# ArchDD/CPP-Raytracer-Rasterizer

Measured on AMD Instinct MI355X. Metric: Mrays/s (primary+shadow), higher is better.
Workload: dtype f32

## Files before the change

cpp-raytracer-rasterizer_amd/capi/binned.cpp:

```cpp
#include "capi.hpp"

namespace mirt {


int PairList::ensure(size_t cap)
{
    int r;
    if ((r = dev_realloc(&d_entries, cap)) || (r = dev_realloc(&d_pair_keys, cap)) || (r = dev_realloc(&d_pair_vals, cap)) ||
        (r = dev_realloc(&d_sorted_keys, cap)) || (r = dev_realloc(&d_tmp_vals, cap))) { cap_entries = 0; return r; }
    cap_entries = (uint32_t)cap;
    return MIRT_OK;
}


void PairList::poll()
{
    if (count_pending && hipEventQuery(ev_count) == hipSuccess) {
        known_pairs = *h_count; have_known = true; count_pending = false;
    }
    (void)hipGetLastError();
}

int PairList::record_count()
{
    if (!count_event_due) return MIRT_OK;
    count_event_due = false;
    HIP_TRY(hipEventRecord(ev_count, g.stream));
    count_pending = true;
    return MIRT_OK;
}

PassPlan KeptPass::plan_for(uint64_t key, int mode, PairList &P) const
{
    static const bool reuse_off = env_int("MIRT_BIN_REUSE", 1) == 0;
    P.poll();
    return kept_pass_plan(bin_key_valid, bin_key == key, P.have_known, P.known_pairs > P.cap_used, last_bin_mode == mode, reuse_off);
}

int bin_pass(PairList &S, BinSet bs, const OriginRow *cam_tab, const OriginRow *light_tab, uint32_t *counter, uint32_t *bin_off,
             uint32_t *npairs, bool may_guess = false)
{
    int rc;
    S.count_event_due = false;
    S.poll();
    const bool guess = may_guess && S.have_known;
    if (!S.d_entries || !S.cap_entries) {
        static const size_t initial = [] { const long v = env_int("MIRT_BIN_INITIAL_PAIRS", 0); return v > 0 ? (size_t)v : (size_t)1 << 20; }();
        if ((rc = S.ensure(initial))) return rc;
    }
    if (bs.nbins > BIN_MAX_KEYS) return fail(MIRT_ERR_INVALID_ARGUMENT, "binning: %u sort keys exceed the %u the bucket sort holds", bs.nbins, BIN_MAX_KEYS);
    bs.chunk_tris = 256;
    const dim3 bin_grid((unsigned)std::min<long long>((long long)((g.n + bs.chunk_tris - 1) / bs.chunk_tris) * bs.nframes, (long long)g.cu_count * 8));
    bs.counters = counter;
    const uint32_t nbuckets = bucket_sort_buckets(bs.nbins);
    if (nbuckets + 1 > S.cap_buckets) {
        if ((rc = dev_grow(&S.d_bucket, &S.cap_buckets, nbuckets + 1, (size_t)3 * (nbuckets + 1), false))) return rc;
        HIP_TRY(hipMemsetAsync(S.d_bucket, 0, sizeof(uint32_t) * 3 * (nbuckets + 1), g.stream));
        S.bucket_dirty = false;
    }
    uint32_t *bcnt = S.d_bucket, *bbase = S.d_bucket + S.cap_buckets, *bcur = S.d_bucket + 2 * (size_t)S.cap_buckets;
    bs.bucket_cnt = bcnt; bs.nbuckets = nbuckets; bs.bucket_shift = bucket_sort_shift(bs.nbins);
    const size_t bin_lds = (size_t)nbuckets * sizeof(uint32_t);
    {
        static const bool once = [] {
            (void)hipFuncSetAttribute(reinterpret_cast<const void *>(&k_bin_pairs<512>), hipFuncAttributeMaxDynamicSharedMemorySize, 48 * 1024);
            (void)hipFuncSetAttribute(reinterpret_cast<const void *>(&k_bin_pairs<256>), hipFuncAttributeMaxDynamicSharedMemorySize, 48 * 1024);
            return true; }();
        (void)once;
    }
    static const int bin_wg_env = (int)env_int("MIRT_BIN_WG", 0);
    const int bin_wg = (bin_wg_env == 256 || bin_wg_env == 512) ? bin_wg_env : ((g.n < 400000 && g.in_flight >= 3) ? 256 : 512);
    if (guess && pairs_wanted(S.known_pairs) > S.cap_entries) {
        HIP_TRY(hipStreamSynchronize(g.stream));
        if ((rc = S.ensure(pairs_grown(pairs_wanted(S.known_pairs))))) return rc;
    }
    bool publish_count = false;
    for (int attempt = 0; attempt < 2; attempt++) {
        static const uint32_t test_cap = [] { const long v = env_int("MIRT_TEST_PAIR_CAP", 0); return v > 0 ? (uint32_t)v : 0u; }();
        S.cap_used = (guess && test_cap && test_cap < S.cap_entries) ? test_cap : S.cap_entries;
        BinPairs pairs = { S.d_pair_keys, S.d_pair_vals, S.cap_used };
        bs.entries = S.d_entries; bs.cap_entries = S.cap_used;
        if (attempt) HIP_TRY(hipMemsetAsync(counter, 0, 4, g.stream));
        if (attempt || S.bucket_dirty) HIP_TRY(hipMemsetAsync(S.d_bucket, 0, sizeof(uint32_t) * 3 * (size_t)S.cap_buckets, g.stream));
        S.bucket_dirty = true;
        if (bin_wg == 256) hipLaunchKernelGGL(k_bin_pairs<256>, bin_grid, dim3(256), bin_lds, g.stream, g.d_tris, cam_tab, light_tab, g.n, bs, pairs);
        else hipLaunchKernelGGL(k_bin_pairs<512>, bin_grid, dim3(512), bin_lds, g.stream, g.d_tris, cam_tab, light_tab, g.n, bs, pairs);
        if (guess) {
            if (!S.h_count) {
                HIP_TRY(hipHostMalloc(reinterpret_cast<void **>(&S.h_count), 64, hipHostMallocDefault));
                HIP_TRY(hipEventCreateWithFlags(&S.ev_count, hipEventDisableTiming));
            }
            if (!S.count_pending) publish_count = true;
            *npairs = S.known_pairs;
            break;
        }
        uint32_t total = 0;
        HIP_TRY(hipStreamSynchronize(g.stream));
        HIP_TRY(hipMemcpy(&total, counter, 4, hipMemcpyDeviceToHost));
        *npairs = total;
        S.known_pairs = total; S.have_known = true;
        S.count_pending = false;
        if (total <= S.cap_entries) break;
        if (attempt == 1) return fail(MIRT_ERR_HIP, "binning produced %u pairs twice with room for %u", total, S.cap_entries);
        if ((rc = S.ensure(pairs_after_readback(total)))) return rc;
    }
#ifdef MIRT_BIN_STATS
    {
        uint32_t c[16];
        (void)hipMemcpy(c, counter, 64, hipMemcpyDeviceToHost);
        fprintf(stderr, "[mirt bin stats] flattened units=%u max per work item=%u direct items=%u | huge: box valid=%u no box=%u (camera frame %u) waves in the joint test=%u\n", c[8], c[9], c[10], c[11], c[12], c[14], c[15]);
        fprintf(stderr, "[mirt bin stats] tris=%d frames=%d  pairs=%u  bins=%u | large items walked=%u level-1 rounds=%u level-2 steps=%u pairs=%u max steps/item=%u items>100 steps=%u\n",
                g.n, bs.nframes, *npairs, bs.nbins, c[2], c[3], c[4], c[5], c[6], c[7]);
        (void)hipMemset(counter + 2, 0, 56);
    }
#endif
    uint32_t *count_out = nullptr;
    if (publish_count) HIP_TRY(hipHostGetDevicePointer(reinterpret_cast<void **>(&count_out), S.h_count, 0));
    HIP_TRY(bucket_sort_pairs(S.d_pair_keys, S.d_pair_vals, counter, S.cap_used, *npairs, bs.nbins, S.d_sorted_keys, S.d_tmp_vals,
                              bcnt, bbase, bcur, bin_off, S.d_entries, g.cu_count, g.stream, count_out));
    S.bucket_dirty = false;
    S.count_event_due = publish_count;
    return MIRT_OK;
}

uint64_t light_key_of(const float *origins, int nlights)
{
    return Fnv(g.scene_version).mix(origins + 3, sizeof(float) * 3 * nlights).mix(&nlights, 4).mix(&g.n, 4).h;
}

int light_shells_for(int nlights, int cube_bins, uint32_t keys_in_front)
{
    static const int env = (int)env_int("MIRT_LIGHT_SHELLS", 0);
    return light_shells_rule(nlights, cube_bins, keys_in_front, env);
}

int ensure_face_lists(LightPass &S, int nlights)
{
    int rc;
    if ((rc = S.ensure_counters(LIGHT_COUNTER_BYTES))) return rc;
    S.d_face_counts = S.d_bin_counters + 128;
    const size_t want = (size_t)6 * (size_t)nlights * (size_t)g.n;
    if (want > S.cap_face_sel && (rc = dev_grow(&S.d_face_sel, &S.cap_face_sel, want, want, true))) return rc;
    return MIRT_OK;
}

static int cube_bin_chain(LightPass &S, const BinFrameDesc *d_frames, const float *d_origins, int nlights, uint32_t nkeys, OriginRow *light_tab,
                          uint32_t *bin_off, uint32_t *counter, uint32_t *npairs, bool may_guess)
{
    hipLaunchKernelGGL(k_select_faces, dim3((unsigned)std::min<long long>(((long long)g.n + 1023) / 1024, (long long)g.cu_count), nlights), dim3(1024), 0, g.stream,
                       g.d_tris, g.n, d_origins, d_frames, light_tab, S.d_face_sel, (uint32_t)g.n, S.d_face_counts);
    BinSet bs;
    memset(&bs, 0, sizeof bs);
    bs.frames = d_frames; bs.nframes = 6 * nlights; bs.nbins = nkeys; bs.bin_off = bin_off;
    bs.face_lists = S.d_face_sel; bs.face_counts = S.d_face_counts; bs.face_stride = (uint32_t)g.n;
    return bin_pass(S.pairs, bs, nullptr, light_tab, counter, bin_off, npairs, may_guess);
}

int light_cache_ensure(LightCache &C, LightPass &S, const float *origins, int nlights, int cube_bins, bool *built)
{
    int rc;
    const uint64_t key = light_key_of(origins, nlights);
    if (built) *built = false;
    if (C.holds(key, cube_bins)) return MIRT_OK;
    if (built) *built = true;
// ... 115 lines not shown
    kept.forget();
    return dev_grow(&d_sel, &sel_n, g.n, (size_t)g.n, true);
}

SelectOut CameraPass::select_out(const OriginTables &T, int count_word) const
{
    SelectOut so;
    memset(&so, 0, sizeof so);
    so.cam_tab = T.d_cam_tab; so.sel = d_sel;
    so.sel_count = d_bin_counters + count_word; so.sel_count_next = d_bin_counters + (count_word ^ 1);
    return so;
}

static void launch_prep_select(const BinFrameDesc &frame, const SelectOut &so)
{
    const unsigned sel_grid = (unsigned)std::min<long long>(((long long)g.n + 1023) / 1024, (long long)g.cu_count);
    if (sel_grid) hipLaunchKernelGGL(k_prep_select, dim3(sel_grid), dim3(1024), 0, g.stream, g.d_tris, g.n, frame, so);
}

int binned_pass(const mirt_view *view, StreamState &ss, const float *origins, int nlights, int y0, int y1, BinnedPass *bp)
{
    int rc;
    CameraPass &S = ss.cam;
    LightPass &L = ss.lt;
    g.stats.mode_used = MIRT_RT_BINNED;
    g.stats_sel_count = nullptr;
    bool fixed_grid = false;
    const int fine_bins = light_cube_bins_for(nlights, &fixed_grid);

    const uint64_t lkey = light_key_of(origins, nlights);
    if (g.lc.track_key == lkey) g.lc.stable++;
    else { g.lc.track_key = lkey; g.lc.stable = 0; }
// ... 97 lines not shown
    CameraPass &S = ss.cam;
    if ((rc = ss.tabs.ensure_cam_rows()) || (rc = S.ensure_sel()) || (rc = S.ensure_counters(512))) return rc;
    S.kept.forget();
    const BinFrameDesc fr = make_camera_frame(view, 0, 0, g.aa);
    SelectOut so = S.select_out(ss.tabs, HIST_SEL_COUNT);
    if ((rc = hist_prepare(ss.hist, fr, &so))) return rc;
    if (!g.hist_armed) return MIRT_OK;
    HIP_TRY(hipMemsetAsync(so.sel_count, 0, 4, g.stream));
    launch_prep_select(fr, so);
    HIP_TRY(hipGetLastError());
    return hist_publish(ss.hist);
}

int binned_trace(const RtFrame &f, StreamState &ss, const BinnedPass &bp)
{
    int rc;
    CameraPass &S = ss.cam;
    RtTraceFrame tf;
    memset(&tf, 0, sizeof tf);
    tf.f = f;
    tf.f.cam_tab = ss.tabs.d_cam_tab;
    tf.f.light_tab = bp.light_tab;
    tf.f.unsafe = nullptr;
    tf.cam_off = bp.cam_off;
    tf.cam_entries = S.pairs.d_entries;
    tf.sel = S.d_sel; tf.sel_count = S.d_bin_counters + SEL_COUNT0 + S.sel_parity;
    static const int lazy_env = (int)env_int("MIRT_LAZY_GEO", -1);
    const bool lazy_geo = lazy_env >= 0 ? (lazy_env != 0) : (g.n >= 400000);
    tf.geo = g.d_geo;
    tf.shade = g.d_shade;
    tf.light_off = bp.cube.light_off;
// ... 17 lines not shown
    const size_t lds = rt_trace_lds_bytes(1);
    k_begin(MIRT_K_TRACE);
    g.pending_counted = g.profiling;
    if (f.aa > 1) {
        if (g.profiling) hipLaunchKernelGGL((k_rt_trace2<true, true>), tgrid, dim3(64), lds, g.stream, tf);
        else hipLaunchKernelGGL((k_rt_trace2<true, false>), tgrid, dim3(64), lds, g.stream, tf);
    } else {
        static const int waves5_env = (int)env_int("MIRT_TR_WAVES5", -1);
        const bool waves5 = waves5_env >= 0 ? (waves5_env != 0) : (g.n >= 400000 || g.in_flight <= 2);
        if (g.profiling) hipLaunchKernelGGL((k_rt_trace2<false, true>), tgrid, dim3(64), lds, g.stream, tf);
        else if (waves5) hipLaunchKernelGGL((k_rt_trace2<false, false, 5>), tgrid, dim3(64), lds, g.stream, tf);
        else hipLaunchKernelGGL((k_rt_trace2<false, false>), tgrid, dim3(64), lds, g.stream, tf);
    }
    k_end(MIRT_K_TRACE);
    HIP_TRY(hipGetLastError());
    return (rc = S.pairs.record_count()) ? rc : ss.lt.pairs.record_count();
}

}
```

cpp-raytracer-rasterizer_amd/capi/capi.hpp:

```cpp
#pragma once

#include "../csrc/bin_sort.hpp"
#include "../csrc/comm.hpp"
#include "../csrc/cull.hpp"
#include "../csrc/dof.hpp"
#include "../csrc/rt_common.hpp"
#include "../csrc/raster_common.hpp"
#include "../csrc/rt_binned.hpp"
#include "../csrc/rt_trace_frame.hpp"
#include "../csrc/scan.hpp"
#include "../query/rt_query.hpp"
#include "../lights/many_lights.hpp"
#include "cube_plan.hpp"
#include "pass_plan.hpp"
#include "object_plan.hpp"
#include "dof_plan.hpp"
#include "env.hpp"

#include <cstdarg>
#include <cstdio>
#include <cstdlib>
#include <cstring>
#include <algorithm>
#include <cmath>
// ... 53 lines not shown
    uint32_t *d_flags = nullptr;

    int ensure_cam_rows();
    void release();
};

struct PairList {
    uint32_t *d_entries = nullptr;
    uint32_t *d_pair_keys = nullptr, *d_pair_vals = nullptr, *d_sorted_keys = nullptr;
    uint32_t *d_tmp_vals = nullptr;
    uint32_t *d_bucket = nullptr;
    uint32_t cap_buckets = 0;
    bool bucket_dirty = false;
    uint32_t cap_entries = 0;
    uint32_t cap_used = 0;
    uint32_t *h_count = nullptr;
    hipEvent_t ev_count = nullptr;
    bool count_pending = false;
    bool count_event_due = false;
    bool have_known = false;
    uint32_t known_pairs = 0;

    int ensure(size_t cap);
    void poll();
    int record_count();
    void forget_scene() { have_known = false; count_pending = false; }
    void release();
};

struct KeptPass {
    uint64_t bin_key = 0;
    bool bin_key_valid = false;
    int last_bin_mode = -1;
    uint32_t bin_entries = 0;

    PassPlan plan_for(uint64_t key, int mode, PairList &P) const;
    void keep(uint64_t key, int mode) { bin_key = key; last_bin_mode = mode; bin_key_valid = true; }
    void forget() { bin_key_valid = false; }
};

// ... 424 lines not shown
```

cpp-raytracer-rasterizer_amd/capi/pass_plan.hpp:

```cpp
#pragma once

#include "../query/rt_query.hpp"
#include "cube_plan.hpp"

#include <cmath>
#include <cstring>

namespace mirt {

struct Fnv {
    uint64_t h;
    explicit Fnv(uint64_t seed) : h(0xcbf29ce484222325ull ^ seed) {}
    Fnv &mix(const void *p, size_t nb) { for (size_t i = 0; i < nb; i++) { h ^= ((const unsigned char *)p)[i]; h *= 0x100000001b3ull; } return *this; }
};

struct PassPlan { bool fresh, may_guess, reuse; };
inline PassPlan kept_pass_plan(bool valid, bool key_equal, bool count_known, bool count_above_cap, bool same_kind, bool reuse_off)
{
    const bool fresh = !valid || !key_equal || (count_known && count_above_cap);
    return PassPlan{ fresh, same_kind, !fresh && !reuse_off };
}

inline size_t pairs_wanted(uint32_t known) { return (size_t)known + known / 2 + 4096; }
inline size_t pairs_grown(size_t want) { return want + want / 4; }
inline size_t pairs_after_readback(uint32_t total) { return (size_t)total + total / 8 + 4096; }

inline int light_shells_rule(int nlights, int cube_bins, uint32_t keys_in_front, int env)
{
    const long long bins = 6ll * cube_bins * cube_bins * std::max(nlights, 1);
    int ns = (env >= 1 && env <= 64) ? env : 16;
    while (ns > 1 && bins * ns + keys_in_front + 64 > (long long)BIN_MAX_KEYS) ns >>= 1;
    return ns;
}
inline int camera_shells_rule(long long tiles, int env)
{
    int ns = (int)std::min<long long>(8, std::max<long long>(1, (4ll << 20) / std::max<long long>(tiles, 1)));
    if (env >= 1 && env <= 64) ns = env;
    while (ns > 1 && tiles * ns + 64 > (long long)BIN_MAX_KEYS) ns >>= 1;
    return ns;
}
// ... 60 lines not shown
```

cpp-raytracer-rasterizer_amd/capi/state.cpp:

```cpp
#include "capi.hpp"

namespace mirt {

int dev_realloc_bytes(void **p, size_t bytes)
{
    if (*p) { (void)hipFree(*p); *p = nullptr; }
    if (bytes == 0) return MIRT_OK;
    hipError_t e = hipMalloc(p, bytes);
    if (e != hipSuccess) { *p = nullptr; return fail(MIRT_ERR_OUT_OF_MEMORY, "hipMalloc(%zu bytes): %s", bytes, hipGetErrorString(e)); }
    return MIRT_OK;
}

int check_frame_args(const mirt_view *view, const mirt_light *lights, int nlights, const float *indirect, const void *xrgb, int pitch_bytes,
                     bool need_scene, int y0, int y1)
{
    int rc;
    if ((rc = need_init())) return rc;
    if (!view || !indirect) return fail(MIRT_ERR_INVALID_ARGUMENT, "view / indirect must not be NULL");
    if (view->width < 1 || view->height < 1 || view->width > 32768 || view->height > 32768)
        return fail(MIRT_ERR_INVALID_ARGUMENT, "frame size %dx%d out of range [1,32768]", view->width, view->height);
    if (nlights < 0 || nlights > MIRT_MAX_LIGHTS) return fail(MIRT_ERR_INVALID_ARGUMENT, "nlights %d out of range [0,%d]", nlights, MIRT_MAX_LIGHTS);
    if (nlights > 0 && !lights) return fail(MIRT_ERR_INVALID_ARGUMENT, "lights must not be NULL when nlights > 0");
    if (need_scene && g.n <= 0) return fail(MIRT_ERR_NO_SCENE, "no scene uploaded (mirt_scene_upload)");
    if (!xrgb) return fail(MIRT_ERR_INVALID_ARGUMENT, "xrgb output must not be NULL");
// ... 32 lines not shown
    memset(ss.ev_used, 0, sizeof ss.ev_used);
    ss.call_timed = g.profiling;
    if (ss.call_timed) (void)hipEventRecord(ss.ev[EV_CALL0], g.stream);
}
void call_end() { if (g.cur().call_timed) (void)hipEventRecord(g.cur().ev[EV_CALL1], g.stream); g.stats_stream = g.stream; g.stats_pending = true; }


static void dev_free(std::initializer_list<void *> ptrs) { for (void *p : ptrs) if (p) (void)hipFree(p); }

void OriginTables::release() { dev_free({ d_cam_tab, d_light_tab, d_origins, d_flags }); *this = OriginTables(); }

void PairList::release()
{
    dev_free({ d_entries, d_pair_keys, d_pair_vals, d_sorted_keys, d_tmp_vals, d_bucket });
    if (h_count) (void)hipHostFree(h_count);
    if (ev_count) (void)hipEventDestroy(ev_count);
    *this = PairList();
}

void CameraPass::release() { pairs.release(); dev_free({ d_bin_off, d_bin_counters, d_frames, d_sel, d_order }); *this = CameraPass(); }

void LightPass::release() { pairs.release(); dev_free({ d_bin_off, d_bin_counters, d_frames, d_face_sel, d_light_tab, d_light_rows }); *this = LightPass(); }

void CostHist::release()
{
    dev_free({ d_hist });
    if (h_hist) (void)hipHostFree(h_hist);
    for (hipEvent_t e : ev_hist) if (e) (void)hipEventDestroy(e);
    *this = CostHist();
}

// ... 67 lines not shown
```

cpp-raytracer-rasterizer_amd/csrc/bin_bucket_sort.hip:

```cpp
#include "bin_sort.hpp"

#include <algorithm>
#include <cstdlib>
#include <type_traits>

namespace mirt {

constexpr int BS_PER_THREAD = 16;
constexpr int BS_CHUNK = 256 * BS_PER_THREAD;
constexpr int BS_LOCAL_PER_THREAD = 16;
constexpr int BS_MAX_SHIFT = 12;
constexpr int BS_MAX_BUCKET_KEYS = 1 << BS_MAX_SHIFT;

__device__ __forceinline__ uint32_t bs_block_scan(uint32_t v, uint32_t *s_wave , uint32_t *total)
{
    const int lane = threadIdx.x & 63, wave = threadIdx.x >> 6;
    uint32_t incl = v;
#pragma unroll
    for (int d = 1; d < 64; d <<= 1) {
        const uint32_t o = __shfl_up(incl, d);
        if (lane >= d) incl += o;
    }
    __syncthreads();
    if (lane == 63) s_wave[wave] = incl;
    __syncthreads();
    uint32_t off = 0, all = 0;
#pragma unroll
    for (int w = 0; w < 4; w++) { if (w < wave) off += s_wave[w]; all += s_wave[w]; }
    *total = all;
    return off + incl - v;
}

__global__ __launch_bounds__(256) void k_bs_scatter(const uint32_t *__restrict__ keys, const uint32_t *__restrict__ vals,
                                                    const uint32_t *__restrict__ total_ptr, uint32_t cap, uint32_t nbuckets, int shift,
                                                    const uint32_t *__restrict__ bucket_cnt, uint32_t *__restrict__ bucket_base,
                                                    uint32_t *__restrict__ cursor, uint32_t *__restrict__ out_keys, uint32_t *__restrict__ out_vals,
                                                    uint32_t *__restrict__ count_out)
{
    extern __shared__ uint32_t s_dyn[];
    __shared__ uint32_t s_wave[4];
    if (count_out && blockIdx.x == 0 && threadIdx.x == 0) *count_out = *total_ptr;
    if (*total_ptr > cap) return;
    uint32_t *s_base = s_dyn, *s_cnt = s_dyn + nbuckets;
    uint32_t carry = 0;
    for (uint32_t b0 = 0; b0 < nbuckets; b0 += 256) {
        const uint32_t b = b0 + threadIdx.x;
        const uint32_t c = b < nbuckets ? bucket_cnt[b] : 0u;
        uint32_t all;
        const uint32_t excl = carry + bs_block_scan(c, s_wave, &all);
        if (b < nbuckets) { s_base[b] = excl; if (blockIdx.x == 0) bucket_base[b] = excl; }
        carry += all;
    }
    if (blockIdx.x == 0 && threadIdx.x == 0) bucket_base[nbuckets] = carry;
    const uint32_t total = min(*total_ptr, cap);
    for (uint32_t base = blockIdx.x * BS_CHUNK; base < total; base += gridDim.x * BS_CHUNK) {
        for (uint32_t b = threadIdx.x; b < nbuckets; b += 256) s_cnt[b] = 0u;
        __syncthreads();
        uint32_t k[BS_PER_THREAD], v[BS_PER_THREAD], rank[BS_PER_THREAD];
#pragma unroll
        for (int j = 0; j < BS_PER_THREAD; j++) {
            const uint32_t i = base + threadIdx.x + 256u * j;
            k[j] = 0xFFFFFFFFu; v[j] = 0u; rank[j] = 0u;
            if (i < total) { k[j] = keys[i]; v[j] = vals[i]; }
        }
#pragma unroll
        for (int j = 0; j < BS_PER_THREAD; j++)
            if (k[j] != 0xFFFFFFFFu) rank[j] = atomicAdd(&s_cnt[k[j] >> shift], 1u);
        __syncthreads();
// ... 54 lines not shown
            if (i < end) { lo[j] = keys[i]; v[j] = vals[i]; }
        });
        bs_rounds<0, BS_LOCAL_PER_THREAD>(rounds, [&](auto jc) {
            constexpr int j = decltype(jc)::value;
            if (lo[j] != 0xFFFFFFFFu) { lo[j] &= mask; rank[j] = atomicAdd(&s_cnt[lo[j]], 1u); }
        });
    } else {
        for (uint32_t i = beg + threadIdx.x; i < end; i += 256) atomicAdd(&s_cnt[keys[i] & mask], 1u);
    }
    __syncthreads();
    uint32_t carry = beg;
    for (uint32_t i0 = 0; i0 < nb; i0 += 256) {
        const uint32_t i = i0 + threadIdx.x;
        const uint32_t c = i < nb ? s_cnt[i] : 0u;
        uint32_t all;
        const uint32_t excl = carry + bs_block_scan(c, s_wave, &all);
        if (i < nb) {
            s_cnt[i] = excl;
            const uint32_t bin = (bucket << shift) + i;
            if (bin <= nbins) bin_off[bin] = excl;
        }
        carry += all;
    }
    __syncthreads();
    if (small) {
        bs_rounds<0, BS_LOCAL_PER_THREAD>(rounds, [&](auto jc) {
            constexpr int j = decltype(jc)::value;
            if (lo[j] != 0xFFFFFFFFu) entries[s_cnt[lo[j]] + rank[j]] = v[j];
        });
    } else {
        for (uint32_t i = beg + threadIdx.x; i < end; i += 256) {
// ... 1 lines not shown
            entries[at] = vals[i];
        }
    }
}

int bucket_sort_shift(uint32_t nbins)
{
    int shift = 8;
    while (shift < BS_MAX_SHIFT && ((nbins + 1u + (1u << shift) - 1u) >> shift) > 1024u) shift++;
    while (shift > 4 && ((nbins + 1u + (1u << shift) - 1u) >> shift) < 512u) shift--;
    return shift;
}
uint32_t bucket_sort_buckets(uint32_t nbins) { const int s = bucket_sort_shift(nbins); return (nbins + 1u + (1u << s) - 1u) >> s; }

hipError_t bucket_sort_pairs(const uint32_t *keys, const uint32_t *vals, const uint32_t *total_ptr, uint32_t cap, uint32_t expected,
                             uint32_t nbins, uint32_t *tmp_keys, uint32_t *tmp_vals, uint32_t *bucket_cnt, uint32_t *bucket_base,
                             uint32_t *cursor, uint32_t *bin_off, uint32_t *entries, int cu_count, hipStream_t stream, uint32_t *count_out)
{
    const int shift = bucket_sort_shift(nbins);
    const uint32_t nbuckets = bucket_sort_buckets(nbins);
    const size_t lds = (size_t)nbuckets * 2 * sizeof(uint32_t);
    uint32_t chunks = (expected + BS_CHUNK - 1) / BS_CHUNK;
    if (chunks < 1) chunks = 1;
    const uint32_t wgs = std::min<uint32_t>(chunks, (uint32_t)cu_count * 2u);
    hipLaunchKernelGGL(k_bs_scatter, dim3(wgs), dim3(256), lds, stream, keys, vals, total_ptr, cap, nbuckets, shift, bucket_cnt, bucket_base,
                       cursor, tmp_keys, tmp_vals, count_out);
    hipLaunchKernelGGL(k_bs_local, dim3(nbuckets), dim3(256), 0, stream, tmp_keys, tmp_vals, total_ptr, cap, bucket_base, nbins, shift, bucket_cnt,
                       cursor, bin_off, entries);
    return hipGetLastError();
}

}
```

cpp-raytracer-rasterizer_amd/csrc/bin_sort.hpp:

```cpp
#pragma once

#include <hip/hip_runtime.h>
#include <cstddef>
#include <cstdint>

namespace mirt {

int bucket_sort_shift(uint32_t nbins);
uint32_t bucket_sort_buckets(uint32_t nbins);
constexpr uint32_t BUCKET_SORT_MAX_BUCKETS = 8192;
hipError_t bucket_sort_pairs(const uint32_t *keys, const uint32_t *vals, const uint32_t *total_ptr, uint32_t cap, uint32_t expected,
                             uint32_t nbins, uint32_t *tmp_keys, uint32_t *tmp_vals, uint32_t *bucket_cnt, uint32_t *bucket_base,
                             uint32_t *cursor, uint32_t *bin_off, uint32_t *entries, int cu_count, hipStream_t stream, uint32_t *count_out = nullptr);

}
```

cpp-raytracer-rasterizer_amd/csrc/rt_binned.hip:

```cpp
#include "rt_binned.hpp"

#include <float.h>

namespace mirt {

constexpr int BIN_L0 = BIN_COARSE * BIN_COARSE;

struct BinItem {
    float A0[4], A1[4], A2[4], Bu[4], Bv[4];
    float lou, hiu, lov, hiv;
};

__device__ __forceinline__ float bcastf(float v, int lane) { return __builtin_bit_cast(float, __builtin_amdgcn_readlane(__builtin_bit_cast(int, v), lane)); }

__device__ __forceinline__ float corner(float s, float lo, float hi) { return fmaxf(s * lo, s * hi); }

__device__ __forceinline__ bool cell_may_hit(const BinItem &u, const float (&A)[4], float I, float J, float K)
{
    bool ok = true;
#pragma unroll
    for (int k = 0; k < 4; k++) ok = ok && (__builtin_fmaf(J, u.Bv[k], __builtin_fmaf(I, u.Bu[k], A[k])) >= 0.0f);
    return ok && (I + K >= u.lou) && (I <= u.hiu) && (J + K >= u.lov) && (J <= u.hiv);
}

// ... 24 lines not shown
#pragma unroll
        for (int j = i + 1; j < 4; j++) {
#pragma unroll
            for (int k = j + 1; k < 4; k++) empty = empty || bin_triple_infeasible(G[i], G[j], G[k], U, V);
#pragma unroll
            for (int sd = 0; sd < 4; sd++) empty = empty || bin_triple_infeasible(G[i], G[j], side[sd], U, V);
        }
    return empty;
}

struct BinFrameGrid { int nbu, fj0, fj1, cells_x, cy0, ncell; uint32_t fbase, nshell; };

constexpr int BIN_PAIR_BUF = 4096;
#ifndef MIRT_BIN_UNIT
#define MIRT_BIN_UNIT 4
#endif
constexpr int BIN_UNIT = MIRT_BIN_UNIT;
static_assert(BIN_UNIT == 2 || BIN_UNIT == 4 || BIN_UNIT == 8, "a unit is 2, 4 or 8 bins");
template <int WG> constexpr int bin_units_per_thread() { return BIN_PAIR_BUF / 2 / (WG * BIN_UNIT) > 0 ? BIN_PAIR_BUF / 2 / (WG * BIN_UNIT) : 1; }
constexpr int BIN_DIRECT_SIDE = 32;

struct BinLargeSink {
    uint32_t *s_keys, *s_vals;
    uint32_t *s_fill;
    uint32_t *s_valid;
    uint32_t *g_count;
    BinPairs out;
    uint32_t *bucket_cnt;
    int bucket_shift;
};
// ... 47 lines not shown
                    if (pass2 && sink.bucket_cnt) atomicAdd(&sink.bucket_cnt[key >> sink.bucket_shift], 1u);
                }
            }
        }
    }
#ifdef MIRT_BIN_STATS
    if (lane == 0) {
        uint32_t *c = sink.g_count;
        atomicAdd(&c[2], 1u); atomicAdd(&c[3], dbg_l1); atomicAdd(&c[4], dbg_steps); atomicAdd(&c[5], dbg_pairs);
        atomicMax(&c[6], dbg_steps);
        if (dbg_steps > 100) atomicAdd(&c[7], 1u);
    }
#endif
}

constexpr int SEL_WG = 1024;
constexpr int SEL_STAGE = 8192;

__global__ __launch_bounds__(SEL_WG) void k_prep_select(const float *__restrict__ tris15, int n, const BinFrameDesc fr, const SelectOut out)
{
    __shared__ uint32_t s_hist[SEL_HIST_MAX];
    __shared__ uint32_t s_sel[SEL_STAGE];
    __shared__ uint32_t s_fill, s_base;
    const int lane = threadIdx.x & 63;
    if (blockIdx.x == 0) {
        if (out.zero_hits)
            for (int g = threadIdx.x; g < HIT_SHARDS * HIT_SHARD_STRIDE; g += SEL_WG) out.zero_hits[g] = 0ull;
        if (out.zero_counter && (threadIdx.x == 0 || (threadIdx.x >= 16 && threadIdx.x < 80))) out.zero_counter[threadIdx.x] = 0u;
        if (threadIdx.x == 0) *out.sel_count_next = 0u;
        if (out.zero_faces && (int)threadIdx.x < out.zero_faces_n) out.zero_faces[threadIdx.x] = 0u;
    }
    if (out.hist && threadIdx.x < SEL_HIST_MAX) s_hist[threadIdx.x] = 0u;
    if (threadIdx.x == 0) s_fill = 0u;
    __syncthreads();
    const v3 S = V3(fr.S[0], fr.S[1], fr.S[2]);
    const int nchunks = (n + SEL_WG - 1) / SEL_WG;
    const int hist_rows = ((fr.nbv - 1) >> out.hist_shift) + 1;
    auto flush = [&]() {
        __syncthreads();
        const uint32_t staged = s_fill;
        if (threadIdx.x == 0 && staged) s_base = atomicAdd(out.sel_count, staged);
        __syncthreads();
        const uint32_t base = s_base;
        for (uint32_t i = threadIdx.x; i < staged; i += SEL_WG) out.sel[base + i] = s_sel[i];
        __syncthreads();
        if (threadIdx.x == 0) s_fill = 0u;
// ... 29 lines not shown
            uint32_t at0 = 0;
            if (lane == 0) at0 = atomicAdd(&s_fill, (uint32_t)__popcll(m));
            at0 = (uint32_t)__builtin_amdgcn_readfirstlane((int)at0);
            if (keep) s_sel[at0 + (uint32_t)__popcll(m & ((1ull << lane) - 1ull))] = (uint32_t)i;
        }
        __syncthreads();
    }
    flush();
    if (out.hist && threadIdx.x < SEL_HIST_MAX) {
        const uint32_t v = s_hist[threadIdx.x];
        if (v && (int)threadIdx.x < hist_rows) atomicAdd(&out.hist[threadIdx.x], v);
    }
}

constexpr int FACE_STAGE = 2048;
__global__ __launch_bounds__(SEL_WG) void k_select_faces(const float *__restrict__ tris15, int n, const float *__restrict__ origins ,
                                                        const BinFrameDesc *__restrict__ faces , OriginRow *__restrict__ light_tab,
                                                        uint32_t *__restrict__ lists, uint32_t stride, uint32_t *__restrict__ face_counts)
{
    __shared__ uint32_t s_sel[6][FACE_STAGE];
    __shared__ uint32_t s_fill[6], s_base[6];
    const int lane = threadIdx.x & 63, k = (int)blockIdx.y;
    if (threadIdx.x < 6) s_fill[threadIdx.x] = 0u;
    __syncthreads();
    const v3 S = ld3(origins + 3 * (1 + k));
    const int nchunks = (n + SEL_WG - 1) / SEL_WG;
    auto flush = [&]() {
        __syncthreads();
        if (threadIdx.x < 6 && s_fill[threadIdx.x]) s_base[threadIdx.x] = atomicAdd(&face_counts[k * 6 + (int)threadIdx.x], s_fill[threadIdx.x]);
        __syncthreads();
#pragma unroll
        for (int f = 0; f < 6; f++) {
            const uint32_t staged = s_fill[f], base = s_base[f];
            uint32_t *dst = lists + (size_t)(k * 6 + f) * stride + base;
            for (uint32_t i = threadIdx.x; i < staged; i += SEL_WG) dst[i] = s_sel[f][i];
        }
        __syncthreads();
        if (threadIdx.x < 6) s_fill[threadIdx.x] = 0u;
        __syncthreads();
    };
    for (int c = blockIdx.x; c < nchunks; c += gridDim.x) {
        uint32_t most = 0;
#pragma unroll
        for (int f = 0; f < 6; f++) most = max(most, s_fill[f]);
        if (most + (uint32_t)SEL_WG > (uint32_t)FACE_STAGE) flush();
        const int i = c * SEL_WG + (int)threadIdx.x;
        uint32_t keep = 0;
        if (i < n) {
            const float *t15 = tris15 + (size_t)15 * i;
            OriginRow r = make_origin_row(t15, S);
            const v3 va = ld3(t15), vb = ld3(t15 + 3), vc = ld3(t15 + 6);
            r.r2.w = origin_far(va, vb, vc, S);
            light_tab[(size_t)k * n + i] = r;
            for (int f = 0; f < 6; f++) {
                PreBox box;
                bool boxed;
                if (frame_may_see(r, va, vb, vc, faces[k * 6 + f], &box, &boxed)) keep |= 1u << f;
            }
        }
#pragma unroll
        for (int f = 0; f < 6; f++) {
// ... 11 lines not shown
}


template <int WG>
__global__ __launch_bounds__(WG) void k_bin_pairs(const float *__restrict__ tris15, const OriginRow *__restrict__ cam_tab,
                                                   const OriginRow *__restrict__ light_tab, int n, BinSet bs, BinPairs out)
{
    extern __shared__ uint32_t s_bucket[];
    __shared__ uint32_t s_keys[BIN_PAIR_BUF], s_vals[BIN_PAIR_BUF];
    __shared__ float4 s_A2[256], s_Bu[256], s_Bv[256], s_box[256];
    __shared__ uint32_t s_org[256];
    __shared__ uint32_t s_ni[256];
    __shared__ uint32_t s_upr[256];
    __shared__ uint32_t s_tri[256];
    __shared__ uint32_t s_pre[257];
    __shared__ uint32_t s_wave[4];
    __shared__ uint32_t s_base, s_fill, s_valid;
    const int lane = threadIdx.x & 63, wave = threadIdx.x >> 6;
    const int chunk_tris = bs.chunk_tris;
    const int nchunks = (n + chunk_tris - 1) / chunk_tris;
    const bool listed = bs.sel != nullptr;
    const uint32_t nsel = listed ? min(*bs.sel_count, (uint32_t)n) : 0u;
    const int cam_chunk = (listed && nsel < 32768u) ? 64 : chunk_tris;
    const int ncam = listed ? (int)((nsel + (uint32_t)cam_chunk - 1u) / (uint32_t)cam_chunk) : 0;
    const int nrest = listed ? bs.nframes - 1 : bs.nframes;
    const bool faces_listed = bs.face_lists != nullptr;
    __shared__ uint32_t s_first[MAX_BIN_FRAMES + 1];
    if (faces_listed) {
        if (threadIdx.x == 0) {
            uint32_t run = 0;
            for (int ff = 0; ff < nrest; ff++) { s_first[ff] = run; run += (min(bs.face_counts[ff], (uint32_t)n) + (uint32_t)chunk_tris - 1u) / (uint32_t)chunk_tris; }
            s_first[nrest] = run;
// ... 246 lines not shown
                    u.Bu[k] = bcastf(it.Bu[k], src); u.Bv[k] = bcastf(it.Bv[k], src);
                }
                u.lou = bcastf(it.lou, src); u.hiu = bcastf(it.hiu, src); u.lov = bcastf(it.lov, src); u.hiv = bcastf(it.hiv, src);
                const uint32_t utri = (uint32_t)__builtin_amdgcn_readlane((int)tri, src);
                const uint32_t ushell = (uint32_t)__builtin_amdgcn_readlane((int)shell, src);
                const unsigned long long ucells = ((unsigned long long)(uint32_t)__builtin_amdgcn_readlane((int)(cells >> 32), src) << 32) | (uint32_t)__builtin_amdgcn_readlane((int)cells, src);
                bin_walk_large(u, utri, ushell, gr, lane, sink, ucells);
            }
        }
        STAMP(st_huge)
    }
#ifdef MIRT_BIN_STAMPS
    st_t = __builtin_amdgcn_s_memtime();
#endif
    flush();
    STAMP(st_flush)
#ifdef MIRT_BIN_STAMPS
    if (threadIdx.x == 0 && (blockIdx.x % 97) == 0)
        printf("wg %d: total %lld | setup %lld prefix %lld rounds %lld (%d) huge %lld flush %lld\n", (int)blockIdx.x, (long long)__builtin_amdgcn_s_memtime() - st_begin,
               st_setup, st_prefix, st_rounds, st_nrounds, st_huge, st_flush);
#endif
}

template __global__ void k_bin_pairs<512>(const float *, const OriginRow *, const OriginRow *, int, BinSet, BinPairs);
template __global__ void k_bin_pairs<256>(const float *, const OriginRow *, const OriginRow *, int, BinSet, BinPairs);

}
```

cpp-raytracer-rasterizer_amd/csrc/rt_binned.hpp:

```cpp
#pragma once

#include "rt_common.hpp"

namespace mirt {

#ifndef MIRT_ORDER_STRIPE_SHIFT
#define MIRT_ORDER_STRIPE_SHIFT 2
#endif
constexpr int ORDER_STRIPE_SHIFT = MIRT_ORDER_STRIPE_SHIFT;
constexpr int BIN_TILE = 8;
constexpr int BIN_COARSE = 8;
constexpr int CUBE_BINS_MIN = 64;
constexpr int MAX_BIN_FRAMES = 1 + 6 * MIRT_MAX_LIGHTS;

struct BinFrameDesc {
    float P0[3], Pu[3], Pv[3];
    float S[3];
    float ru[3], rv[3], rw[3];
    float ulo, vlo, du, dv;
    float pad_lo, pad_hi;
    float dmax;
    int nbu, nbv;
    int j0, j1;
    uint32_t base;
// ... 16 lines not shown

struct GeoRow { float4 g0, g1, g2; };
struct ShadeRow { float4 n, col; };
typedef OriginRow LightRow;

struct BinSet {
    const BinFrameDesc *frames;
    BinFrameDesc frame0;
    int nframes;
    uint32_t nbins;
    uint32_t *bin_off;
    uint32_t *entries;
    uint32_t cap_entries;
    uint32_t *counters;
    uint32_t *bucket_cnt;
    uint32_t nbuckets;
    int bucket_shift;
    int chunk_tris;
    const uint32_t *sel;
    const uint32_t *sel_count;
    const uint32_t *face_lists;
    const uint32_t *face_counts;
    uint32_t face_stride;
};

constexpr int SEL_HIST_MAX = 256;
struct SelectOut {
    OriginRow *cam_tab;
    uint32_t *sel;
    uint32_t *sel_count;
    uint32_t *sel_count_next;
    uint32_t *hist;
    int hist_shift;
    uint32_t *zero_faces;
    int zero_faces_n;
    unsigned long long *zero_hits;
    uint32_t *zero_counter;
};

struct BinPairs {
    uint32_t *keys;
// ... 225 lines not shown
```

Measured before the change: 57120.

## Fold bucket base scan into last binning workgroup and poll pair count via serial word

```diff
diff --git a/cpp-raytracer-rasterizer_amd/capi/binned.cpp b/cpp-raytracer-rasterizer_amd/capi/binned.cpp
--- a/cpp-raytracer-rasterizer_amd/capi/binned.cpp
+++ b/cpp-raytracer-rasterizer_amd/capi/binned.cpp
@@ -15,19 +15,11 @@
 
 void PairList::poll()
 {
-    if (count_pending && hipEventQuery(ev_count) == hipSuccess) {
-        known_pairs = *h_count; have_known = true; count_pending = false;
-    }
-    (void)hipGetLastError();
-}
-
-int PairList::record_count()
-{
-    if (!count_event_due) return MIRT_OK;
-    count_event_due = false;
-    HIP_TRY(hipEventRecord(ev_count, g.stream));
-    count_pending = true;
-    return MIRT_OK;
+    if (!count_pending) return;
+    const unsigned long long w = __atomic_load_n(h_count, __ATOMIC_ACQUIRE);
+    if (count_serial_accepts(count_word_serial(w), serial)) {
+        known_pairs = count_word_pairs(w); have_known = true; count_pending = false;
+    }
 }
 
 PassPlan KeptPass::plan_for(uint64_t key, int mode, PairList &P) const
@@ -41,7 +33,6 @@
              uint32_t *npairs, bool may_guess = false)
 {
     int rc;
-    S.count_event_due = false;
     S.poll();
     const bool guess = may_guess && S.have_known;
     if (!S.d_entries || !S.cap_entries) {
@@ -59,7 +50,7 @@
         S.bucket_dirty = false;
     }
     uint32_t *bcnt = S.d_bucket, *bbase = S.d_bucket + S.cap_buckets, *bcur = S.d_bucket + 2 * (size_t)S.cap_buckets;
-    bs.bucket_cnt = bcnt; bs.nbuckets = nbuckets; bs.bucket_shift = bucket_sort_shift(bs.nbins);
+    bs.bucket_cnt = bcnt; bs.bucket_base = bbase; bs.nbuckets = nbuckets; bs.bucket_shift = bucket_sort_shift(bs.nbins);
     const size_t bin_lds = (size_t)nbuckets * sizeof(uint32_t);
     {
         static const bool once = [] {
@@ -88,7 +79,7 @@
         if (guess) {
             if (!S.h_count) {
                 HIP_TRY(hipHostMalloc(reinterpret_cast<void **>(&S.h_count), 64, hipHostMallocDefault));
-                HIP_TRY(hipEventCreateWithFlags(&S.ev_count, hipEventDisableTiming));
+                memset(S.h_count, 0, 64);
             }
             if (!S.count_pending) publish_count = true;
             *npairs = S.known_pairs;
@@ -114,12 +105,15 @@
         (void)hipMemset(counter + 2, 0, 56);
     }
 #endif
-    uint32_t *count_out = nullptr;
-    if (publish_count) HIP_TRY(hipHostGetDevicePointer(reinterpret_cast<void **>(&count_out), S.h_count, 0));
+    unsigned long long *count_out = nullptr;
+    if (publish_count) {
+        HIP_TRY(hipHostGetDevicePointer(reinterpret_cast<void **>(&count_out), S.h_count, 0));
+        S.serial++;
+        S.count_pending = true;
+    }
     HIP_TRY(bucket_sort_pairs(S.d_pair_keys, S.d_pair_vals, counter, S.cap_used, *npairs, bs.nbins, S.d_sorted_keys, S.d_tmp_vals,
-                              bcnt, bbase, bcur, bin_off, S.d_entries, g.cu_count, g.stream, count_out));
+                              bcnt, bbase, bcur, bin_off, S.d_entries, g.cu_count, g.stream, count_out, S.serial));
     S.bucket_dirty = false;
-    S.count_event_due = publish_count;
     return MIRT_OK;
 }
 
@@ -147,7 +141,7 @@
 static int cube_bin_chain(LightPass &S, const BinFrameDesc *d_frames, const float *d_origins, int nlights, uint32_t nkeys, OriginRow *light_tab,
                           uint32_t *bin_off, uint32_t *counter, uint32_t *npairs, bool may_guess)
 {
-    hipLaunchKernelGGL(k_select_faces, dim3((unsigned)std::min<long long>(((long long)g.n + 1023) / 1024, (long long)g.cu_count), nlights), dim3(1024), 0, g.stream,
+    hipLaunchKernelGGL(k_select_faces, dim3((unsigned)std::min<long long>(((long long)g.n + FACE_WG - 1) / FACE_WG, (long long)g.cu_count), nlights), dim3(FACE_WG), 0, g.stream,
                        g.d_tris, g.n, d_origins, d_frames, light_tab, S.d_face_sel, (uint32_t)g.n, S.d_face_counts);
     BinSet bs;
     memset(&bs, 0, sizeof bs);
@@ -293,8 +287,8 @@
 
 static void launch_prep_select(const BinFrameDesc &frame, const SelectOut &so)
 {
-    const unsigned sel_grid = (unsigned)std::min<long long>(((long long)g.n + 1023) / 1024, (long long)g.cu_count);
-    if (sel_grid) hipLaunchKernelGGL(k_prep_select, dim3(sel_grid), dim3(1024), 0, g.stream, g.d_tris, g.n, frame, so);
+    const unsigned sel_grid = (unsigned)std::min<long long>(((long long)g.n + SEL_WG - 1) / SEL_WG, (long long)g.cu_count * SEL_WGS_PER_CU);
+    if (sel_grid) hipLaunchKernelGGL(k_prep_select, dim3(sel_grid), dim3(SEL_WG), 0, g.stream, g.d_tris, g.n, frame, so);
 }
 
 int binned_pass(const mirt_view *view, StreamState &ss, const float *origins, int nlights, int y0, int y1, BinnedPass *bp)
@@ -422,7 +416,6 @@
 
 int binned_trace(const RtFrame &f, StreamState &ss, const BinnedPass &bp)
 {
-    int rc;
     CameraPass &S = ss.cam;
     RtTraceFrame tf;
     memset(&tf, 0, sizeof tf);
@@ -470,7 +463,7 @@
     }
     k_end(MIRT_K_TRACE);
     HIP_TRY(hipGetLastError());
-    return (rc = S.pairs.record_count()) ? rc : ss.lt.pairs.record_count();
-}
-
-}
+    return MIRT_OK;
+}
+
+}
diff --git a/cpp-raytracer-rasterizer_amd/capi/capi.hpp b/cpp-raytracer-rasterizer_amd/capi/capi.hpp
--- a/cpp-raytracer-rasterizer_amd/capi/capi.hpp
+++ b/cpp-raytracer-rasterizer_amd/capi/capi.hpp
@@ -91,16 +91,14 @@
     bool bucket_dirty = false;
     uint32_t cap_entries = 0;
     uint32_t cap_used = 0;
-    uint32_t *h_count = nullptr;
-    hipEvent_t ev_count = nullptr;
+    unsigned long long *h_count = nullptr;
+    uint32_t serial = 0;
     bool count_pending = false;
-    bool count_event_due = false;
     bool have_known = false;
     uint32_t known_pairs = 0;
 
     int ensure(size_t cap);
     void poll();
-    int record_count();
     void forget_scene() { have_known = false; count_pending = false; }
     void release();
 };
diff --git a/cpp-raytracer-rasterizer_amd/capi/pass_plan.hpp b/cpp-raytracer-rasterizer_amd/capi/pass_plan.hpp
--- a/cpp-raytracer-rasterizer_amd/capi/pass_plan.hpp
+++ b/cpp-raytracer-rasterizer_amd/capi/pass_plan.hpp
@@ -24,6 +24,16 @@
 inline size_t pairs_wanted(uint32_t known) { return (size_t)known + known / 2 + 4096; }
 inline size_t pairs_grown(size_t want) { return want + want / 4; }
 inline size_t pairs_after_readback(uint32_t total) { return (size_t)total + total / 8 + 4096; }
+
+enum class CountSerial { stale, wanted, newer };
+inline CountSerial count_serial_seen(uint32_t published, uint32_t wanted)
+{
+    const int32_t ahead = (int32_t)(published - wanted);
+    return ahead < 0 ? CountSerial::stale : (ahead == 0 ? CountSerial::wanted : CountSerial::newer);
+}
+inline bool count_serial_accepts(uint32_t published, uint32_t wanted) { return count_serial_seen(published, wanted) != CountSerial::stale; }
+inline uint32_t count_word_pairs(unsigned long long w) { return (uint32_t)(w & 0xFFFFFFFFull); }
+inline uint32_t count_word_serial(unsigned long long w) { return (uint32_t)(w >> 32); }
 
 inline int light_shells_rule(int nlights, int cube_bins, uint32_t keys_in_front, int env)
 {
diff --git a/cpp-raytracer-rasterizer_amd/capi/state.cpp b/cpp-raytracer-rasterizer_amd/capi/state.cpp
--- a/cpp-raytracer-rasterizer_amd/capi/state.cpp
+++ b/cpp-raytracer-rasterizer_amd/capi/state.cpp
@@ -70,7 +70,6 @@
 {
     dev_free({ d_entries, d_pair_keys, d_pair_vals, d_sorted_keys, d_tmp_vals, d_bucket });
     if (h_count) (void)hipHostFree(h_count);
-    if (ev_count) (void)hipEventDestroy(ev_count);
     *this = PairList();
 }
 
diff --git a/cpp-raytracer-rasterizer_amd/csrc/bin_bucket_sort.hip b/cpp-raytracer-rasterizer_amd/csrc/bin_bucket_sort.hip
--- a/cpp-raytracer-rasterizer_amd/csrc/bin_bucket_sort.hip
+++ b/cpp-raytracer-rasterizer_amd/csrc/bin_bucket_sort.hip
@@ -6,52 +6,29 @@
 
 namespace mirt {
 
-constexpr int BS_PER_THREAD = 16;
+#ifndef MIRT_BS_PER_THREAD
+#define MIRT_BS_PER_THREAD 16
+#endif
+constexpr int BS_PER_THREAD = MIRT_BS_PER_THREAD;
+static_assert(BS_PER_THREAD == 4 || BS_PER_THREAD == 8 || BS_PER_THREAD == 16, "a thread of k_bs_scatter takes 4, 8 or 16 pairs per chunk");
 constexpr int BS_CHUNK = 256 * BS_PER_THREAD;
 constexpr int BS_LOCAL_PER_THREAD = 16;
 constexpr int BS_MAX_SHIFT = 12;
 constexpr int BS_MAX_BUCKET_KEYS = 1 << BS_MAX_SHIFT;
 
-__device__ __forceinline__ uint32_t bs_block_scan(uint32_t v, uint32_t *s_wave , uint32_t *total)
-{
-    const int lane = threadIdx.x & 63, wave = threadIdx.x >> 6;
-    uint32_t incl = v;
-#pragma unroll
-    for (int d = 1; d < 64; d <<= 1) {
-        const uint32_t o = __shfl_up(incl, d);
-        if (lane >= d) incl += o;
-    }
-    __syncthreads();
-    if (lane == 63) s_wave[wave] = incl;
-    __syncthreads();
-    uint32_t off = 0, all = 0;
-#pragma unroll
-    for (int w = 0; w < 4; w++) { if (w < wave) off += s_wave[w]; all += s_wave[w]; }
-    *total = all;
-    return off + incl - v;
-}
 
 __global__ __launch_bounds__(256) void k_bs_scatter(const uint32_t *__restrict__ keys, const uint32_t *__restrict__ vals,
                                                     const uint32_t *__restrict__ total_ptr, uint32_t cap, uint32_t nbuckets, int shift,
-                                                    const uint32_t *__restrict__ bucket_cnt, uint32_t *__restrict__ bucket_base,
+                                                    const uint32_t *__restrict__ bucket_base,
                                                     uint32_t *__restrict__ cursor, uint32_t *__restrict__ out_keys, uint32_t *__restrict__ out_vals,
-                                                    uint32_t *__restrict__ count_out)
+                                                    unsigned long long *__restrict__ count_out, uint32_t serial)
 {
     extern __shared__ uint32_t s_dyn[];
-    __shared__ uint32_t s_wave[4];
-    if (count_out && blockIdx.x == 0 && threadIdx.x == 0) *count_out = *total_ptr;
+    if (count_out && blockIdx.x == 0 && threadIdx.x == 0)
+        __hip_atomic_store(count_out, (unsigned long long)*total_ptr | ((unsigned long long)serial << 32), __ATOMIC_RELEASE, __HIP_MEMORY_SCOPE_SYSTEM);
     if (*total_ptr > cap) return;
     uint32_t *s_base = s_dyn, *s_cnt = s_dyn + nbuckets;
-    uint32_t carry = 0;
-    for (uint32_t b0 = 0; b0 < nbuckets; b0 += 256) {
-        const uint32_t b = b0 + threadIdx.x;
-        const uint32_t c = b < nbuckets ? bucket_cnt[b] : 0u;
-        uint32_t all;
-        const uint32_t excl = carry + bs_block_scan(c, s_wave, &all);
-        if (b < nbuckets) { s_base[b] = excl; if (blockIdx.x == 0) bucket_base[b] = excl; }
-        carry += all;
-    }
-    if (blockIdx.x == 0 && threadIdx.x == 0) bucket_base[nbuckets] = carry;
+    for (uint32_t b = threadIdx.x; b < nbuckets; b += 256) s_base[b] = bucket_base[b];
     const uint32_t total = min(*total_ptr, cap);
     for (uint32_t base = blockIdx.x * BS_CHUNK; base < total; base += gridDim.x * BS_CHUNK) {
         for (uint32_t b = threadIdx.x; b < nbuckets; b += 256) s_cnt[b] = 0u;
@@ -136,7 +113,7 @@
         const uint32_t i = i0 + threadIdx.x;
         const uint32_t c = i < nb ? s_cnt[i] : 0u;
         uint32_t all;
-        const uint32_t excl = carry + bs_block_scan(c, s_wave, &all);
+        const uint32_t excl = carry + bs_block_scan<256>(c, s_wave, &all);
         if (i < nb) {
             s_cnt[i] = excl;
             const uint32_t bin = (bucket << shift) + i;
@@ -168,8 +145,9 @@
 uint32_t bucket_sort_buckets(uint32_t nbins) { const int s = bucket_sort_shift(nbins); return (nbins + 1u + (1u << s) - 1u) >> s; }
 
 hipError_t bucket_sort_pairs(const uint32_t *keys, const uint32_t *vals, const uint32_t *total_ptr, uint32_t cap, uint32_t expected,
-                             uint32_t nbins, uint32_t *tmp_keys, uint32_t *tmp_vals, uint32_t *bucket_cnt, uint32_t *bucket_base,
-                             uint32_t *cursor, uint32_t *bin_off, uint32_t *entries, int cu_count, hipStream_t stream, uint32_t *count_out)
+                             uint32_t nbins, uint32_t *tmp_keys, uint32_t *tmp_vals, uint32_t *bucket_cnt, const uint32_t *bucket_base,
+                             uint32_t *cursor, uint32_t *bin_off, uint32_t *entries, int cu_count, hipStream_t stream,
+                             unsigned long long *count_out, uint32_t serial)
 {
     const int shift = bucket_sort_shift(nbins);
     const uint32_t nbuckets = bucket_sort_buckets(nbins);
@@ -177,8 +155,8 @@
     uint32_t chunks = (expected + BS_CHUNK - 1) / BS_CHUNK;
     if (chunks < 1) chunks = 1;
     const uint32_t wgs = std::min<uint32_t>(chunks, (uint32_t)cu_count * 2u);
-    hipLaunchKernelGGL(k_bs_scatter, dim3(wgs), dim3(256), lds, stream, keys, vals, total_ptr, cap, nbuckets, shift, bucket_cnt, bucket_base,
-                       cursor, tmp_keys, tmp_vals, count_out);
+    hipLaunchKernelGGL(k_bs_scatter, dim3(wgs), dim3(256), lds, stream, keys, vals, total_ptr, cap, nbuckets, shift, bucket_base,
+                       cursor, tmp_keys, tmp_vals, count_out, serial);
     hipLaunchKernelGGL(k_bs_local, dim3(nbuckets), dim3(256), 0, stream, tmp_keys, tmp_vals, total_ptr, cap, bucket_base, nbins, shift, bucket_cnt,
                        cursor, bin_off, entries);
     return hipGetLastError();
diff --git a/cpp-raytracer-rasterizer_amd/csrc/bin_sort.hpp b/cpp-raytracer-rasterizer_amd/csrc/bin_sort.hpp
--- a/cpp-raytracer-rasterizer_amd/csrc/bin_sort.hpp
+++ b/cpp-raytracer-rasterizer_amd/csrc/bin_sort.hpp
@@ -10,7 +10,59 @@
 uint32_t bucket_sort_buckets(uint32_t nbins);
 constexpr uint32_t BUCKET_SORT_MAX_BUCKETS = 8192;
 hipError_t bucket_sort_pairs(const uint32_t *keys, const uint32_t *vals, const uint32_t *total_ptr, uint32_t cap, uint32_t expected,
-                             uint32_t nbins, uint32_t *tmp_keys, uint32_t *tmp_vals, uint32_t *bucket_cnt, uint32_t *bucket_base,
-                             uint32_t *cursor, uint32_t *bin_off, uint32_t *entries, int cu_count, hipStream_t stream, uint32_t *count_out = nullptr);
+                             uint32_t nbins, uint32_t *tmp_keys, uint32_t *tmp_vals, uint32_t *bucket_cnt, const uint32_t *bucket_base,
+                             uint32_t *cursor, uint32_t *bin_off, uint32_t *entries, int cu_count, hipStream_t stream,
+                             unsigned long long *count_out = nullptr, uint32_t serial = 0);
+
+constexpr int BIN_DONE_WORD = 1;
+
+#ifdef __HIPCC__
+template <int WG>
+__device__ __forceinline__ uint32_t bs_block_scan(uint32_t v, uint32_t *s_wave , uint32_t *total)
+{
+    const int lane = threadIdx.x & 63, wave = threadIdx.x >> 6;
+    uint32_t incl = v;
+#pragma unroll
+    for (int d = 1; d < 64; d <<= 1) {
+        const uint32_t o = __shfl_up(incl, d);
+        if (lane >= d) incl += o;
+    }
+    __syncthreads();
+    if (lane == 63) s_wave[wave] = incl;
+    __syncthreads();
+    uint32_t off = 0, all = 0;
+#pragma unroll
+    for (int w = 0; w < WG / 64; w++) { if (w < wave) off += s_wave[w]; all += s_wave[w]; }
+    *total = all;
+    return off + incl - v;
+}
+
+template <int WG>
+__device__ __forceinline__ void bs_scan_bucket_bases(const uint32_t *bucket_cnt, uint32_t *bucket_base, uint32_t nbuckets, uint32_t *s_wave )
+{
+    if (nbuckets <= 4u * WG) {
+        const uint32_t b0 = 4u * threadIdx.x;
+        uint32_t c[4];
+#pragma unroll
+        for (uint32_t q = 0; q < 4; q++) c[q] = b0 + q < nbuckets ? __hip_atomic_load(&bucket_cnt[b0 + q], __ATOMIC_RELAXED, __HIP_MEMORY_SCOPE_AGENT) : 0u;
+        uint32_t all;
+        uint32_t run = bs_block_scan<WG>(c[0] + c[1] + c[2] + c[3], s_wave, &all);
+#pragma unroll
+        for (uint32_t q = 0; q < 4; q++) { if (b0 + q < nbuckets) bucket_base[b0 + q] = run; run += c[q]; }
+        if (threadIdx.x == 0) bucket_base[nbuckets] = all;
+        return;
+    }
+    uint32_t carry = 0;
+    for (uint32_t b0 = 0; b0 < nbuckets; b0 += WG) {
+        const uint32_t b = b0 + threadIdx.x;
+        const uint32_t c = b < nbuckets ? __hip_atomic_load(&bucket_cnt[b], __ATOMIC_RELAXED, __HIP_MEMORY_SCOPE_AGENT) : 0u;
+        uint32_t all;
+        const uint32_t excl = carry + bs_block_scan<WG>(c, s_wave, &all);
+        if (b < nbuckets) bucket_base[b] = excl;
+        carry += all;
+    }
+    if (threadIdx.x == 0) bucket_base[nbuckets] = carry;
+}
+#endif
 
 }
diff --git a/cpp-raytracer-rasterizer_amd/csrc/rt_binned.hip b/cpp-raytracer-rasterizer_amd/csrc/rt_binned.hip
--- a/cpp-raytracer-rasterizer_amd/csrc/rt_binned.hip
+++ b/cpp-raytracer-rasterizer_amd/csrc/rt_binned.hip
@@ -1,4 +1,5 @@
 #include "rt_binned.hpp"
+#include "bin_sort.hpp"
 
 #include <float.h>
 
@@ -62,6 +63,9 @@
 constexpr int BIN_PAIR_BUF = 4096;
 #ifndef MIRT_BIN_UNIT
 #define MIRT_BIN_UNIT 4
+#endif
+#ifndef MIRT_BIN_DONE_FENCE
+#define MIRT_BIN_DONE_FENCE 0
 #endif
 constexpr int BIN_UNIT = MIRT_BIN_UNIT;
 static_assert(BIN_UNIT == 2 || BIN_UNIT == 4 || BIN_UNIT == 8, "a unit is 2, 4 or 8 bins");
@@ -139,8 +143,7 @@
 #endif
 }
 
-constexpr int SEL_WG = 1024;
-constexpr int SEL_STAGE = 8192;
+constexpr int SEL_STAGE = 8 * SEL_WG;
 
 __global__ __launch_bounds__(SEL_WG) void k_prep_select(const float *__restrict__ tris15, int n, const BinFrameDesc fr, const SelectOut out)
 {
@@ -151,10 +154,12 @@
     if (blockIdx.x == 0) {
         if (out.zero_hits)
             for (int g = threadIdx.x; g < HIT_SHARDS * HIT_SHARD_STRIDE; g += SEL_WG) out.zero_hits[g] = 0ull;
-        if (out.zero_counter && (threadIdx.x == 0 || (threadIdx.x >= 16 && threadIdx.x < 80))) out.zero_counter[threadIdx.x] = 0u;
+        if (out.zero_counter && (threadIdx.x <= (unsigned)BIN_DONE_WORD || (threadIdx.x >= 16 && threadIdx.x < 80))) out.zero_counter[threadIdx.x] = 0u;
         if (threadIdx.x == 0) *out.sel_count_next = 0u;
-        if (out.zero_faces && (int)threadIdx.x < out.zero_faces_n) out.zero_faces[threadIdx.x] = 0u;
-    }
+        if (out.zero_faces)
+            for (int q = threadIdx.x; q < out.zero_faces_n; q += SEL_WG) out.zero_faces[q] = 0u;
+    }
+    static_assert(SEL_WG >= SEL_HIST_MAX && SEL_WG >= 80, "a thread per histogram row, and per counter word block 0 zeroes");
     if (out.hist && threadIdx.x < SEL_HIST_MAX) s_hist[threadIdx.x] = 0u;
     if (threadIdx.x == 0) s_fill = 0u;
     __syncthreads();
@@ -214,7 +219,7 @@
 }
 
 constexpr int FACE_STAGE = 2048;
-__global__ __launch_bounds__(SEL_WG) void k_select_faces(const float *__restrict__ tris15, int n, const float *__restrict__ origins ,
+__global__ __launch_bounds__(FACE_WG) void k_select_faces(const float *__restrict__ tris15, int n, const float *__restrict__ origins ,
                                                         const BinFrameDesc *__restrict__ faces , OriginRow *__restrict__ light_tab,
                                                         uint32_t *__restrict__ lists, uint32_t stride, uint32_t *__restrict__ face_counts)
 {
@@ -224,7 +229,7 @@
     if (threadIdx.x < 6) s_fill[threadIdx.x] = 0u;
     __syncthreads();
     const v3 S = ld3(origins + 3 * (1 + k));
-    const int nchunks = (n + SEL_WG - 1) / SEL_WG;
+    const int nchunks = (n + FACE_WG - 1) / FACE_WG;
     auto flush = [&]() {
         __syncthreads();
         if (threadIdx.x < 6 && s_fill[threadIdx.x]) s_base[threadIdx.x] = atomicAdd(&face_counts[k * 6 + (int)threadIdx.x], s_fill[threadIdx.x]);
@@ -233,7 +238,7 @@
         for (int f = 0; f < 6; f++) {
             const uint32_t staged = s_fill[f], base = s_base[f];
             uint32_t *dst = lists + (size_t)(k * 6 + f) * stride + base;
-            for (uint32_t i = threadIdx.x; i < staged; i += SEL_WG) dst[i] = s_sel[f][i];
+            for (uint32_t i = threadIdx.x; i < staged; i += FACE_WG) dst[i] = s_sel[f][i];
         }
         __syncthreads();
         if (threadIdx.x < 6) s_fill[threadIdx.x] = 0u;
@@ -243,8 +248,8 @@
         uint32_t most = 0;
 #pragma unroll
         for (int f = 0; f < 6; f++) most = max(most, s_fill[f]);
-        if (most + (uint32_t)SEL_WG > (uint32_t)FACE_STAGE) flush();
-        const int i = c * SEL_WG + (int)threadIdx.x;
+        if (most + (uint32_t)FACE_WG > (uint32_t)FACE_STAGE) flush();
+        const int i = c * FACE_WG + (int)threadIdx.x;
         uint32_t keep = 0;
         if (i < n) {
             const float *t15 = tris15 + (size_t)15 * i;
@@ -286,8 +291,8 @@
     __shared__ uint32_t s_upr[256];
     __shared__ uint32_t s_tri[256];
     __shared__ uint32_t s_pre[257];
-    __shared__ uint32_t s_wave[4];
-    __shared__ uint32_t s_base, s_fill, s_valid;
+    __shared__ uint32_t s_wave[WG / 64 > 4 ? WG / 64 : 4];
+    __shared__ uint32_t s_base, s_fill, s_valid, s_last;
     const int lane = threadIdx.x & 63, wave = threadIdx.x >> 6;
     const int chunk_tris = bs.chunk_tris;
     const int nchunks = (n + chunk_tris - 1) / chunk_tris;
@@ -564,6 +569,23 @@
     st_t = __builtin_amdgcn_s_memtime();
 #endif
     flush();
+    if (bs.bucket_cnt) {
+        asm volatile("s_waitcnt vmcnt(0)" ::: "memory");
+        __syncthreads();
+        if (threadIdx.x == 0) {
+#if MIRT_BIN_DONE_FENCE
+            __threadfence();
+#endif
+            const uint32_t done = atomicAdd(&bs.counters[BIN_DONE_WORD], 1u);
+            s_last = done == gridDim.x - 1u;
+            if (s_last) bs.counters[BIN_DONE_WORD] = 0u;
+        }
+        __syncthreads();
+        if (s_last) {
+            __builtin_amdgcn_fence(__ATOMIC_ACQUIRE, "agent");
+            bs_scan_bucket_bases<WG>(bs.bucket_cnt, bs.bucket_base, bs.nbuckets, s_wave);
+        }
+    }
     STAMP(st_flush)
 #ifdef MIRT_BIN_STAMPS
     if (threadIdx.x == 0 && (blockIdx.x % 97) == 0)
diff --git a/cpp-raytracer-rasterizer_amd/csrc/rt_binned.hpp b/cpp-raytracer-rasterizer_amd/csrc/rt_binned.hpp
--- a/cpp-raytracer-rasterizer_amd/csrc/rt_binned.hpp
+++ b/cpp-raytracer-rasterizer_amd/csrc/rt_binned.hpp
@@ -54,6 +54,7 @@
     uint32_t cap_entries;
     uint32_t *counters;
     uint32_t *bucket_cnt;
+    uint32_t *bucket_base;
     uint32_t nbuckets;
     int bucket_shift;
     int chunk_tris;
@@ -65,6 +66,16 @@
 };
 
 constexpr int SEL_HIST_MAX = 256;
+#ifndef MIRT_SEL_WG
+#define MIRT_SEL_WG 1024
+#endif
+#ifndef MIRT_SEL_WGS_PER_CU
+#define MIRT_SEL_WGS_PER_CU 1
+#endif
+constexpr int SEL_WG = MIRT_SEL_WG;
+constexpr int SEL_WGS_PER_CU = MIRT_SEL_WGS_PER_CU;
+static_assert(SEL_WG == 256 || SEL_WG == 512 || SEL_WG == 1024, "k_prep_select runs in workgroups of 256, 512 or 1024 threads");
+constexpr int FACE_WG = 1024;
 struct SelectOut {
     OriginRow *cam_tab;
     uint32_t *sel;
```

Result: slower. 56480 (-1.1%).
